# 0xPolygonZero/plonky2

Measured on AMD Instinct MI355X. Metric: LDE+Poseidon-commit GFE/s, higher is better.
Workload: dtype u64 (Goldilocks)

## Files before the change

### plonky2_amd/csrc/gl_mul3.hpp

```cpp
#pragma once
#include "asm_block.h"
#include "gl.hpp"

namespace gl {

#define P2_SA "v[70:71]", "v70", "v71", "v[72:73]", "v72", "v73", "v[74:75]", "v74", "v75", "s[40:41]", "s[42:43]"
#define P2_SB "v[76:77]", "v76", "v77", "v[78:79]", "v78", "v79", "v[80:81]", "v80", "v81", "s[44:45]", "s[46:47]"
#define P2_SC "v[82:83]", "v82", "v83", "v[84:85]", "v84", "v85", "v[86:87]", "v86", "v87", "s[48:49]", "s[50:51]"

#define P2_ST1(P, P0, P1, M, M0, M1, Q, Q0, Q1, C1, C2, a0, a1, b0, b1, r0, r1) "v_mad_u64_u32 " P ", " C1 ", %[" a0 "], %[" b0 "], 0\n\t"
#define P2_ST2(P, P0, P1, M, M0, M1, Q, Q0, Q1, C1, C2, a0, a1, b0, b1, r0, r1) "v_mad_u64_u32 " M ", " C1 ", %[" a1 "], %[" b0 "], 0\n\t"
#define P2_ST3(P, P0, P1, M, M0, M1, Q, Q0, Q1, C1, C2, a0, a1, b0, b1, r0, r1) "v_mad_u64_u32 " M ", " C2 ", %[" a0 "], %[" b1 "], " M "\n\t"
#define P2_ST4(P, P0, P1, M, M0, M1, Q, Q0, Q1, C1, C2, a0, a1, b0, b1, r0, r1) "v_mad_u64_u32 " Q ", " C1 ", %[" a1 "], %[" b1 "], 0\n\t"
#define P2_ST5(P, P0, P1, M, M0, M1, Q, Q0, Q1, C1, C2, a0, a1, b0, b1, r0, r1) "v_add_co_u32 " P1 ", " C1 ", " P1 ", " M0 "\n\t"
#define P2_ST6(P, P0, P1, M, M0, M1, Q, Q0, Q1, C1, C2, a0, a1, b0, b1, r0, r1) "v_addc_co_u32 " Q0 ", " C1 ", " Q0 ", " M1 ", " C1 "\n\t"
#define P2_ST7(P, P0, P1, M, M0, M1, Q, Q0, Q1, C1, C2, a0, a1, b0, b1, r0, r1) "v_addc_co_u32 " Q1 ", " C1 ", " Q1 ", 0, " C1 "\n\t"
#define P2_ST8(P, P0, P1, M, M0, M1, Q, Q0, Q1, C1, C2, a0, a1, b0, b1, r0, r1) "v_subb_co_u32 " P0 ", " C1 ", " P0 ", " Q1 ", " C2 "\n\t"
#define P2_ST9(P, P0, P1, M, M0, M1, Q, Q0, Q1, C1, C2, a0, a1, b0, b1, r0, r1) "v_subb_co_u32 " P1 ", " C1 ", " P1 ", 0, " C1 "\n\t"
#define P2_ST10(P, P0, P1, M, M0, M1, Q, Q0, Q1, C1, C2, a0, a1, b0, b1, r0, r1) "v_mad_u64_u32 " P ", " C2 ", " Q0 ", -1, " P "\n\t"
#define P2_ST11(P, P0, P1, M, M0, M1, Q, Q0, Q1, C1, C2, a0, a1, b0, b1, r0, r1) "v_cndmask_b32 " M0 ", 0, 1, " C2 "\n\t"
#define P2_ST12(P, P0, P1, M, M0, M1, Q, Q0, Q1, C1, C2, a0, a1, b0, b1, r0, r1) "v_subb_co_u32 " M0 ", " C1 ", " M0 ", 0, " C1 "\n\t"
#define P2_ST13(P, P0, P1, M, M0, M1, Q, Q0, Q1, C1, C2, a0, a1, b0, b1, r0, r1) "v_add_u32 " P1 ", " P1 ", " M0 "\n\t"
#define P2_ST14(P, P0, P1, M, M0, M1, Q, Q0, Q1, C1, C2, a0, a1, b0, b1, r0, r1) "v_mad_i64_i32 %[" r0 "], " C1 ", " M0 ", -1, " P "\n\t"

// ... 151 lines not shown
           (P2_CF_CLOBBERS3));
    r[0] = ra;
    r[1] = rb;
    r[2] = rc;
}

#define P2_CA1(ST) P2_APPLY(ST, P2_CA, "xa0", "xa1", "ya0", "ya1", "ra0")
__device__ __forceinline__ u64 mul1cf(u64 a, u64 b) {
    if (!P2_ASM_INTERPRETED()) return mul(a, b);
    u64 ra;
    P2_ASM(P2_CA1(P2_CF0) P2_CA1(P2_CF1) P2_CA1(P2_CF2) P2_CA1(P2_CF3) P2_CA1(P2_CF4) P2_CA1(P2_CF5) P2_CA1(P2_CF6) P2_CA1(P2_CF7)
               P2_CA1(P2_CF8) P2_CA1(P2_CF9) P2_NOP P2_CA1(P2_CF10) P2_CA1(P2_CF11) P2_NOP P2_CA1(P2_CF12) P2_CA1(P2_CF13)
                   P2_CA1(P2_CF14) P2_CA1(P2_CF15),
           (P2_O([ra0], "=&v", ra)),
           (P2_I([xa0], "v", (u32)a), P2_I([xa1], "v", (u32)(a >> 32)), P2_I([ya0], "v", (u32)b), P2_I([ya1], "v", (u32)(b >> 32))),
           ("v70", "v71", "v72", "v73", "v74", "v75", "v76", "v77", "s40", "s41", "s42", "s43"));
    return ra;
}

#define P2_CG0(P, P0, P1, M, M0, M1, N, N0, N1, T, T0, T1, C1, C2, a0, a1, b0, b1, r0) "v_mov_b32 " T1 ", 0\n\t"
#define P2_CG1(P, P0, P1, M, M0, M1, N, N0, N1, T, T0, T1, C1, C2, a0, a1, b0, b1, r0) "v_mad_u64_u32 " P ", " C1 ", %[" a0 "], %[" b0 "], 0\n\t"
#define P2_CG2(P, P0, P1, M, M0, M1, N, N0, N1, T, T0, T1, C1, C2, a0, a1, b0, b1, r0) "v_mov_b32 " T0 ", " P1 "\n\t"
#define P2_CG3(P, P0, P1, M, M0, M1, N, N0, N1, T, T0, T1, C1, C2, a0, a1, b0, b1, r0) "v_mad_u64_u32 " M ", " C1 ", %[" a1 "], %[" b0 "], " T "\n\t"
#define P2_CG4(P, P0, P1, M, M0, M1, N, N0, N1, T, T0, T1, C1, C2, a0, a1, b0, b1, r0) "v_mad_u64_u32 " N ", " C2 ", %[" a0 "], %[" b1 "], " M "\n\t"
#define P2_CG5(P, P0, P1, M, M0, M1, N, N0, N1, T, T0, T1, C1, C2, a0, a1, b0, b1, r0) "v_mov_b32 " T0 ", " N1 "\n\t"
#define P2_CG6(P, P0, P1, M, M0, M1, N, N0, N1, T, T0, T1, C1, C2, a0, a1, b0, b1, r0) "v_mad_u64_u32 " T ", " C1 ", %[" a1 "], %[" b1 "], " T "\n\t"
#define P2_CG7(P, P0, P1, M, M0, M1, N, N0, N1, T, T0, T1, C1, C2, a0, a1, b0, b1, r0) "v_subb_co_u32 " M0 ", " C1 ", " P0 ", " T1 ", " C2 "\n\t"
#define P2_CG8 P2_CF10
#define P2_CG9 P2_CF11
#define P2_CG10 P2_CF12
#define P2_CG11 P2_CF13
#define P2_CG12 P2_CF14
#define P2_CG13 P2_CF15

__device__ __forceinline__ void mul3cg(const u64 a[3], const u64 b[3], u64 r[3]) {
    if (!P2_ASM_INTERPRETED()) {
        for (int k = 0; k < 3; ++k) r[k] = mul(a[k], b[k]);
        return;
    }
    u64 ra, rb, rc;
    P2_ASM(P2_CROW(P2_CG0) P2_CROW(P2_CG1) P2_CROW(P2_CG2) P2_CROW(P2_CG3) P2_CROW(P2_CG4) P2_CROW(P2_CG5) P2_CROW(P2_CG6) P2_CROW(P2_CG7)
               P2_CROW(P2_CG8) P2_CROW(P2_CG9) P2_CROW(P2_CG10) P2_CROW(P2_CG11) P2_CROW(P2_CG12) P2_CROW(P2_CG13),
           (P2_O([ra0], "=&v", ra), P2_O([rb0], "=&v", rb), P2_O([rc0], "=&v", rc)),
           (P2_I([xa0], "v", (u32)a[0]), P2_I([xa1], "v", (u32)(a[0] >> 32)), P2_I([ya0], "v", (u32)b[0]),
            P2_I([ya1], "v", (u32)(b[0] >> 32)), P2_I([xb0], "v", (u32)a[1]), P2_I([xb1], "v", (u32)(a[1] >> 32)),
            P2_I([yb0], "v", (u32)b[1]), P2_I([yb1], "v", (u32)(b[1] >> 32)), P2_I([xc0], "v", (u32)a[2]),
            P2_I([xc1], "v", (u32)(a[2] >> 32)), P2_I([yc0], "v", (u32)b[2]), P2_I([yc1], "v", (u32)(b[2] >> 32))),
           (P2_CF_CLOBBERS3));
    r[0] = ra;
    r[1] = rb;
    r[2] = rc;
}

#define P2_HT "v[76:77]", "v76", "v77"
#define P2_HA "v[70:71]", "v70", "v71", "v[72:73]", "v72", "v73", "v[74:75]", "v74", "v75", P2_HT, "s[40:41]", "s[42:43]"
#define P2_HB "v[78:79]", "v78", "v79", "v[80:81]", "v80", "v81", "v[82:83]", "v82", "v83", P2_HT, "s[44:45]", "s[46:47]"
#define P2_HC "v[86:87]", "v86", "v87", "v[88:89]", "v88", "v89", "v[90:91]", "v90", "v91", P2_HT, "s[48:49]", "s[50:51]"
#define P2_CH23(...) P2_CG2(__VA_ARGS__) P2_CG3(__VA_ARGS__)
#define P2_CH6(P, P0, P1, M, M0, M1, N, N0, N1, T, T0, T1, C1, C2, a0, a1, b0, b1, r0) "v_mad_u64_u32 " M ", " C1 ", %[" a1 "], %[" b1 "], " T "\n\t"
#define P2_CH56(...) P2_CG5(__VA_ARGS__) P2_CH6(__VA_ARGS__)
#define P2_CH7(P, P0, P1, M, M0, M1, N, N0, N1, T, T0, T1, C1, C2, a0, a1, b0, b1, r0) "v_subb_co_u32 " P0 ", " C1 ", " P0 ", " M1 ", " C2 "\n\t"
#define P2_CH8(P, P0, P1, M, M0, M1, N, N0, N1, T, T0, T1, C1, C2, a0, a1, b0, b1, r0) "v_subb_co_u32 " P1 ", " C1 ", " N0 ", 0, " C1 "\n\t"
#define P2_CH9(P, P0, P1, M, M0, M1, N, N0, N1, T, T0, T1, C1, C2, a0, a1, b0, b1, r0) "v_mad_u64_u32 " P ", " C2 ", " M0 ", -1, " P "\n\t"
#define P2_CH12(P, P0, P1, M, M0, M1, N, N0, N1, T, T0, T1, C1, C2, a0, a1, b0, b1, r0) "v_add_u32 " P1 ", " P1 ", " N0 "\n\t"
#define P2_CH13(P, P0, P1, M, M0, M1, N, N0, N1, T, T0, T1, C1, C2, a0, a1, b0, b1, r0) "v_mad_i64_i32 %[" r0 "], " C1 ", " N0 ", -1, " P "\n\t"
#define P2_HROW(ST)                                          \
    P2_APPLY(ST, P2_HA, "xa0", "xa1", "ya0", "ya1", "ra0")   \
    P2_APPLY(ST, P2_HB, "xb0", "xb1", "yb0", "yb1", "rb0")   \
    P2_APPLY(ST, P2_HC, "xc0", "xc1", "yc0", "yc1", "rc0")
__device__ __forceinline__ void mul3ch(const u64 a[3], const u64 b[3], u64 r[3]) {
    if (!P2_ASM_INTERPRETED()) {
        for (int k = 0; k < 3; ++k) r[k] = mul(a[k], b[k]);
        return;
    }
    u64 ra, rb, rc;
    P2_ASM("v_mov_b32 v77, 0\n\t" P2_HROW(P2_CG1) P2_HROW(P2_CH23) P2_HROW(P2_CG4) P2_HROW(P2_CH56) P2_HROW(P2_CH7) P2_HROW(P2_CH8)
               P2_HROW(P2_CH9) P2_HROW(P2_CG10) P2_HROW(P2_CG11) P2_HROW(P2_CH12) P2_HROW(P2_CH13),
           (P2_O([ra0], "=&v", ra), P2_O([rb0], "=&v", rb), P2_O([rc0], "=&v", rc)),
           (P2_I([xa0], "v", (u32)a[0]), P2_I([xa1], "v", (u32)(a[0] >> 32)), P2_I([ya0], "v", (u32)b[0]),
            P2_I([ya1], "v", (u32)(b[0] >> 32)), P2_I([xb0], "v", (u32)a[1]), P2_I([xb1], "v", (u32)(a[1] >> 32)),
            P2_I([yb0], "v", (u32)b[1]), P2_I([yb1], "v", (u32)(b[1] >> 32)), P2_I([xc0], "v", (u32)a[2]),
            P2_I([xc1], "v", (u32)(a[2] >> 32)), P2_I([yc0], "v", (u32)b[2]), P2_I([yc1], "v", (u32)(b[2] >> 32))),
           ("v70", "v71", "v72", "v73", "v74", "v75", "v76", "v77", "v78", "v79", "v80", "v81", "v82", "v83", "v86", "v87", "v88", "v89",
            "v90", "v91", "s40", "s41", "s42", "s43", "s44", "s45", "s46", "s47", "s48", "s49", "s50", "s51"));
    r[0] = ra;
    r[1] = rb;
    r[2] = rc;
}

__device__ __forceinline__ u64 mul1cg(u64 a, u64 b) {
    if (!P2_ASM_INTERPRETED()) return mul(a, b);
    u64 ra;
    P2_ASM(P2_CA1(P2_CG0) P2_CA1(P2_CG1) P2_CA1(P2_CG2) P2_CA1(P2_CG3) P2_CA1(P2_CG4) P2_CA1(P2_CG5) P2_CA1(P2_CG6) P2_CA1(P2_CG7) P2_NOP
               P2_CA1(P2_CG8) P2_CA1(P2_CG9) P2_NOP P2_CA1(P2_CG10) P2_CA1(P2_CG11) P2_CA1(P2_CG12) P2_CA1(P2_CG13),
           (P2_O([ra0], "=&v", ra)),
           (P2_I([xa0], "v", (u32)a), P2_I([xa1], "v", (u32)(a >> 32)), P2_I([ya0], "v", (u32)b), P2_I([ya1], "v", (u32)(b >> 32))),
           ("v70", "v71", "v72", "v73", "v74", "v75", "v76", "v77", "s40", "s41", "s42", "s43"));
    return ra;
}

#define P2_FD1(P, P0, P1, M, M0, M1, Q, Q0, Q1, C1, C2, a0, a1, b0, b1, r0, r1) "v_mad_u64_u32 " P ", " C1 ", %[" b1 "], -1, %[" a0 "]\n\t"
#define P2_FD2(P, P0, P1, M, M0, M1, Q, Q0, Q1, C1, C2, a0, a1, b0, b1, r0, r1) "v_add_co_u32 " P1 ", " C1 ", " P1 ", %[" b0 "]\n\t"
#define P2_FD3(P, P0, P1, M, M0, M1, Q, Q0, Q1, C1, C2, a0, a1, b0, b1, r0, r1) "v_cndmask_b32 " M0 ", 0, -1, " C1 "\n\t"
#define P2_FD4(P, P0, P1, M, M0, M1, Q, Q0, Q1, C1, C2, a0, a1, b0, b1, r0, r1) "v_mad_u64_u32 %[" r0 "], " C1 ", " M0 ", 1, " P "\n\t"

__host__ __device__ __forceinline__ u64 fold_row_c(u64 al, u64 ah) {
    u32 k1;
    u32 w1 = addc32((u32)(al >> 32), (u32)ah, 0u, &k1);
    u32 w2 = (u32)(ah >> 32) + k1;
    u64 lo64 = ((u64)w1 << 32) | (u32)al;
    u64 t = (u64)w2 * 0xFFFFFFFFu + lo64;
    return fold_carry(t, t < lo64);
}

__device__ __forceinline__ void fold3(const u64 al[3], const u64 ah[3], u64 y[3]) {
    if (!P2_ASM_INTERPRETED()) {
        for (int k = 0; k < 3; ++k) y[k] = fold_row_c(al[k], ah[k]);
        return;
    }
    u64 ra, rb, rc;
    P2_ASM(P2_ROW(P2_FD1) P2_ROW(P2_FD2) P2_ROW(P2_FD3) P2_ROW(P2_FD4),
           (P2_O([ra0], "=&v", ra), P2_O([rb0], "=&v", rb), P2_O([rc0], "=&v", rc)),
           (P2_I([xa0], "v", al[0]), P2_I([ya0], "v", (u32)ah[0]), P2_I([ya1], "v", (u32)(ah[0] >> 32)),
            P2_I([xb0], "v", al[1]), P2_I([yb0], "v", (u32)ah[1]), P2_I([yb1], "v", (u32)(ah[1] >> 32)),
            P2_I([xc0], "v", al[2]), P2_I([yc0], "v", (u32)ah[2]), P2_I([yc1], "v", (u32)(ah[2] >> 32))),
           ("v70", "v71", "v72", "v76", "v77", "v78", "v82", "v83", "v84", "s40", "s41", "s44", "s45", "s48", "s49"));
    y[0] = ra;
    y[1] = rb;
    y[2] = rc;
}
__device__ __forceinline__ void fold2(const u64 al[2], const u64 ah[2], u64 y[2]) {
    if (!P2_ASM_INTERPRETED()) {
        for (int k = 0; k < 2; ++k) y[k] = fold_row_c(al[k], ah[k]);
        return;
    }
    u64 ra, rb;
    P2_ASM(P2_ROW2(P2_FD1) P2_ROW2(P2_FD2) P2_NOP0 P2_ROW2(P2_FD3) P2_ROW2(P2_FD4),
           (P2_O([ra0], "=&v", ra), P2_O([rb0], "=&v", rb)),
           (P2_I([xa0], "v", al[0]), P2_I([ya0], "v", (u32)ah[0]), P2_I([ya1], "v", (u32)(ah[0] >> 32)),
            P2_I([xb0], "v", al[1]), P2_I([yb0], "v", (u32)ah[1]), P2_I([yb1], "v", (u32)(ah[1] >> 32))),
           ("v70", "v71", "v72", "v76", "v77", "v78", "s40", "s41", "s44", "s45"));
    y[0] = ra;
    y[1] = rb;
}
__device__ __forceinline__ u64 fold1(u64 al, u64 ah) {
    if (!P2_ASM_INTERPRETED()) return fold_row_c(al, ah);
    u64 ra;
    P2_ASM(P2_A1(P2_FD1, P2_SA) P2_A1(P2_FD2, P2_SA) P2_NOP P2_A1(P2_FD3, P2_SA) P2_A1(P2_FD4, P2_SA),
           (P2_O([ra0], "=&v", ra)), (P2_I([xa0], "v", al), P2_I([ya0], "v", (u32)ah), P2_I([ya1], "v", (u32)(ah >> 32))),
           ("v70", "v71", "v72", "s40", "s41"));
    return ra;
}

}
```

### plonky2_amd/csrc/merkle.hpp

```cpp
#pragma once
#include "poseidon.hpp"
#include "poseidon4.hpp"
#include "poseidon16.hpp"
#include "ntt.hpp"

namespace merkle {
using gl::u32;
using gl::u64;

struct ColMajorReader {
    const u64 *m;
    size_t stride;
    __device__ __forceinline__ u64 operator()(size_t L, unsigned e) const { return m[(size_t)e * stride + L]; }
};
struct RowMajorReader {
    const u64 *m;
    size_t W;
    __device__ __forceinline__ u64 operator()(size_t L, unsigned e) const { return m[L * W + e]; }
};
struct FriPlanarReader {
    const u64 *p0, *p1;
    unsigned arity_bits;
    __device__ __forceinline__ u64 operator()(size_t L, unsigned e) const {
        const u64 *p = (e & 1) ? p1 : p0;
// ... 108 lines not shown
            }
            poseidon4::permute_quad(w, q);
        }
    }
    if (live) {
        u64 *dst = node_slot(digests, cap, h, 0, L);
        if (q == 0) {
            dst[0] = gl::canon(w[0]);
            dst[1] = gl::canon(w[1]);
            dst[2] = gl::canon(w[2]);
        } else if (q == 1) {
            dst[3] = gl::canon(w[0]);
        }
    }
}

__global__ void __launch_bounds__(256) merkle_level_quad_kernel(u64 *digests, u64 *cap, unsigned h, unsigned level,
                                                               size_t n_nodes) {
    const size_t j = ((size_t)blockIdx.x * blockDim.x + threadIdx.x) >> 2;
    const unsigned q = threadIdx.x & 3;
    const bool live = j < n_nodes;
    const u64 *ch = node_slot(digests, cap, h, level - 1, 2 * (live ? j : 0));
    u64 w[3];
#pragma unroll
    for (unsigned u = 0; u < 3; ++u) w[u] = (live && 3 * q + u < 8) ? ch[3 * q + u] : 0;
    poseidon4::permute_quad(w, q);
    if (live) {
        u64 *dst = node_slot(digests, cap, h, level, j);
        if (q == 0) {
            dst[0] = gl::canon(w[0]);
            dst[1] = gl::canon(w[1]);
            dst[2] = gl::canon(w[2]);
        } else if (q == 1) {
            dst[3] = gl::canon(w[0]);
        }
    }
}

template <class Reader>
__global__ void __launch_bounds__(256) hash_leaves_row_kernel(Reader rd, unsigned W, size_t leaf_offset, size_t leaf_count,
                                                             unsigned h, u64 *digests, u64 *cap) {
    const size_t t = ((size_t)blockIdx.x * blockDim.x + threadIdx.x) >> 4;
    const unsigned r = threadIdx.x & 15;
    const bool live = t < leaf_count;
    const size_t L = leaf_offset + (live ? t : 0);
    u64 w = 0;
    if (W <= 4) {
        if (live && r < W) w = rd(L, r);
    } else {
        const poseidon16::RowConsts k = poseidon16::row_consts(r);
        for (unsigned off = 0; off < W; off += 8) {
            const unsigned cnt = W - off < 8 ? W - off : 8;
            if (live && r < cnt) w = rd(L, off + r);
            poseidon16::permute_row(w, r, k);
        }
    }
    if (live && r < 4) node_slot(digests, cap, h, 0, L)[r] = gl::canon(w);
}

__global__ void __launch_bounds__(256) merkle_level_row_kernel(u64 *digests, u64 *cap, unsigned h, unsigned level, size_t n_nodes) {
    const size_t j = ((size_t)blockIdx.x * blockDim.x + threadIdx.x) >> 4;
    const unsigned r = threadIdx.x & 15;
    const bool live = j < n_nodes;
    const u64 *ch = node_slot(digests, cap, h, level - 1, 2 * (live ? j : 0));
    u64 w = (live && r < 8) ? ch[r] : 0;
    const poseidon16::RowConsts k = poseidon16::row_consts(r);
    poseidon16::permute_row(w, r, k);
    if (live && r < 4) node_slot(digests, cap, h, level, j)[r] = gl::canon(w);
}

__global__ void __launch_bounds__(256) permute_batch_row_kernel(u64 *states, size_t count) {
    const size_t t = ((size_t)blockIdx.x * blockDim.x + threadIdx.x) >> 4;
    const unsigned r = threadIdx.x & 15;
    const bool live = t < count && r < 12;
    u64 w = live ? states[12 * t + r] : 0;
    const poseidon16::RowConsts k = poseidon16::row_consts(r);
    poseidon16::permute_row(w, r, k);
    if (live) states[12 * t + r] = gl::canon(w);
}

__global__ void permute_batch_kernel(u64 *states, size_t count) {
    size_t t = (size_t)blockIdx.x * blockDim.x + threadIdx.x;
    if (t >= count) return;
    u64 s[12];
#pragma unroll
    for (int i = 0; i < 12; ++i) s[i] = states[12 * t + i];
    poseidon::permute(s);
#pragma unroll
    for (int i = 0; i < 12; ++i) states[12 * t + i] = gl::canon(s[i]);
}

__global__ void field_selftest_kernel(const u64 *a, const u64 *b, size_t count, u64 *out) {
    size_t t = (size_t)blockIdx.x * blockDim.x + threadIdx.x;
    if (t >= count) return;
    const u64 x = a[t], y = b[t];
    out[t] = gl::canon(gl::mul(x, y));
    out[count + t] = gl::canon(gl::mul1(x, y));
    u64 aa[3] = {x, y, x}, bb[3] = {y, x, x}, rr[3];
    gl::mul3(aa, bb, rr);
    u64 ok = (gl::canon(rr[1]) == gl::canon(rr[0])) && (gl::canon(rr[2]) == gl::canon(gl::mul(x, x))) ? 0 : 1;
    if (gl::canon(gl::mul1_lowregs(x, y)) != gl::canon(gl::mul(x, y))) ok |= 2;
#define P2_CHK_POW2(S)                                                                                              \
    if (gl::canon(ntt::mul_pow2_asm<S>(x)) != gl::canon(gl::mul(x, (S) < 64 ? 1ull << ((S) & 63) : 0xFFFFFFFFull << (((S) - 64) & 31)))) \
        ok |= 4;
    P2_CHK_POW2(12) P2_CHK_POW2(24) P2_CHK_POW2(36) P2_CHK_POW2(48) P2_CHK_POW2(60) P2_CHK_POW2(72) P2_CHK_POW2(84)
    P2_CHK_POW2(1) P2_CHK_POW2(31) P2_CHK_POW2(33) P2_CHK_POW2(63) P2_CHK_POW2(65) P2_CHK_POW2(95)
#undef P2_CHK_POW2
    {
        const u64 al = x >> 1, ah = y >> 1;
        const u64 want = gl::canon(gl::add(al, gl::mul(ah, 1ull << 32)));
        if (gl::canon(gl::fold1(al, ah)) != want) ok |= 8;
        const u64 al3[3] = {al, ah, al ^ 0x2AAAAAAAAAAAAAAAull}, ah3[3] = {ah, al, ah};
        u64 y3[3];
        gl::fold3(al3, ah3, y3);
        for (int k = 0; k < 3; ++k)
            if (gl::canon(y3[k]) != gl::canon(gl::add(al3[k], gl::mul(ah3[k], 1ull << 32)))) ok |= 16;
    }
    {
        const u64 a2[2] = {x, y ^ 0x9E3779B97F4A7C15ull}, b2[2] = {y, x};
        u64 r2[2];
        gl::mul2(a2, b2, r2);
        if (gl::canon(r2[0]) != gl::canon(gl::mul(x, y)) || gl::canon(r2[1]) != gl::canon(gl::mul(a2[1], x))) ok |= 32;
        const u64 l2[2] = {x >> 1, y >> 1}, h2[2] = {y >> 1, x >> 1};
        u64 f2[2];
        gl::fold2(l2, h2, f2);
        for (int k = 0; k < 2; ++k)
            if (gl::canon(f2[k]) != gl::canon(gl::add(l2[k], gl::mul(h2[k], 1ull << 32)))) ok |= 64;
    }
    if (gl::canon(gl::mul_add(x, y, x ^ y)) != gl::canon(gl::add(gl::mul(x, y), x ^ y)) || gl::canon(gl::mul_add(y, x, ~0ull)) != gl::canon(gl::add(gl::mul(x, y), ~0ull)) ||
        gl::canon(gl::mul_add(x, x, y)) != gl::canon(gl::add(gl::mul(x, x), y)))
        ok |= 128;
    {
        const u64 a3[3] = {x, y, x}, b3[3] = {y, x, x}, c3[3] = {x ^ y, ~0ull, y};
        u64 r3[3];
        gl::mad3(a3, b3, c3, r3);
        for (int k = 0; k < 3; ++k)
            if (gl::canon(r3[k]) != gl::canon(gl::add(gl::mul(a3[k], b3[k]), c3[k]))) ok |= 256;
    }
    {
        const u64 a3[3] = {x, y, x ^ 0x9E3779B97F4A7C15ull}, b3[3] = {y, y, x};
        u64 r3[3];
        gl::mul3cf(a3, b3, r3);
        for (int k = 0; k < 3; ++k)
            if (gl::canon(r3[k]) != gl::canon(gl::mul(a3[k], b3[k]))) ok |= 512;
        if (gl::canon(gl::mul1cf(x, y)) != gl::canon(gl::mul(x, y)) || gl::canon(gl::mul1cf(y, y)) != gl::canon(gl::mul(y, y))) ok |= 512;
        gl::mul3cg(a3, b3, r3);
        for (int k = 0; k < 3; ++k)
            if (gl::canon(r3[k]) != gl::canon(gl::mul(a3[k], b3[k]))) ok |= 512;
        gl::mul3ch(a3, b3, r3);
        for (int k = 0; k < 3; ++k)
            if (gl::canon(r3[k]) != gl::canon(gl::mul(a3[k], b3[k]))) ok |= 512;
        if (gl::canon(gl::mul1cg(x, y)) != gl::canon(gl::mul(x, y)) || gl::canon(gl::mul1cg(y, y)) != gl::canon(gl::mul(y, y))) ok |= 512;
    }
    out[2 * count + t] = gl::canon(rr[0]);
    out[5 * count + t] = ok;
    out[3 * count + t] = gl::canon(gl::add(x, y));
    out[4 * count + t] = gl::canon(gl::sub(x, y));
}

}
```

### plonky2_amd/csrc/poseidon.hpp

```cpp
#pragma once
#include "gl.hpp"
#include "gl_mul3.hpp"
#ifndef P2HOT_EMU
#define P2_CONST_QUAL __constant__
#endif
#define P2_LITERAL_QUAL static constexpr
#include "poseidon_constants.h"

namespace poseidon {
using gl::u32;
using gl::u64;

#define RC P2_POSEIDON_ALL_ROUND_CONSTANTS
#define RC_SPLIT P2_POSEIDON_PUSHED_ROUND_CONSTANTS_SPLIT

__device__ __forceinline__ u64 sbox7(u64 x) {
    u64 x2 = gl::sqr(x);
    u64 x4 = gl::sqr(x2);
    u64 x3 = gl::mul(x, x2);
    return gl::mul(x3, x4);
}

#ifndef P2HOT_SBOX_CF
#define P2HOT_SBOX_CF 2
// ... 67 lines not shown
        ah[0] += (u64)h0 * C;
        al[1] += (u64)l1 * C;
        ah[1] += (u64)h1 * C;
        al[2] += (u64)l2 * C;
        ah[2] += (u64)h2 * C;
        return;
    }
    u64 d;
    P2_ASM_NC("v_mad_u64_u32 %0, %6, %7, %13, %0\n\t"
              "v_mad_u64_u32 %1, %6, %8, %13, %1\n\t"
              "v_mad_u64_u32 %2, %6, %9, %13, %2\n\t"
              "v_mad_u64_u32 %3, %6, %10, %13, %3\n\t"
              "v_mad_u64_u32 %4, %6, %11, %13, %4\n\t"
              "v_mad_u64_u32 %5, %6, %12, %13, %5",
              (P2_O(, "+v", al[0]), P2_O(, "+v", ah[0]), P2_O(, "+v", al[1]), P2_O(, "+v", ah[1]), P2_O(, "+v", al[2]),
               P2_O(, "+v", ah[2]), P2_O(, "=&s", d)),
              (P2_I(, "v", l0), P2_I(, "v", h0), P2_I(, "v", l1), P2_I(, "v", h1), P2_I(, "v", l2), P2_I(, "v", h2),
               P2_I(, "n", C)));
}
template <bool HAS_K>
__device__ __forceinline__ void mds_first(u64 (&al)[3], u64 (&ah)[3], u32 l0, u32 h0, u32 l1, u32 h1, u32 l2, u32 h2,
                                          const u64 *k) {
    if (!P2_ASM_INTERPRETED()) {
        const u64 z[6] = {0, 0, 0, 0, 0, 0};
        const u64 *kk = HAS_K ? k : z;
        al[0] = (u64)l0 * 17u + kk[0];
        ah[0] = (u64)h0 * 17u + kk[1];
        al[1] = (u64)l1 * 17u + kk[2];
        ah[1] = (u64)h1 * 17u + kk[3];
        al[2] = (u64)l2 * 17u + kk[4];
        ah[2] = (u64)h2 * 17u + kk[5];
        return;
    }
    u64 d;
    if (HAS_K) {
        P2_ASM_NC("v_mad_u64_u32 %0, %6, %7, 17, %13\n\t"
                  "v_mad_u64_u32 %1, %6, %8, 17, %14\n\t"
                  "v_mad_u64_u32 %2, %6, %9, 17, %15\n\t"
                  "v_mad_u64_u32 %3, %6, %10, 17, %16\n\t"
                  "v_mad_u64_u32 %4, %6, %11, 17, %17\n\t"
                  "v_mad_u64_u32 %5, %6, %12, 17, %18",
                  (P2_O(, "=&v", al[0]), P2_O(, "=&v", ah[0]), P2_O(, "=&v", al[1]), P2_O(, "=&v", ah[1]),
                   P2_O(, "=&v", al[2]), P2_O(, "=&v", ah[2]), P2_O(, "=&s", d)),
                  (P2_I(, "v", l0), P2_I(, "v", h0), P2_I(, "v", l1), P2_I(, "v", h1), P2_I(, "v", l2), P2_I(, "v", h2),
                   P2_I(, "s", k[0]), P2_I(, "s", k[1]), P2_I(, "s", k[2]), P2_I(, "s", k[3]), P2_I(, "s", k[4]),
                   P2_I(, "s", k[5])));
    } else {
        P2_ASM_NC("v_mad_u64_u32 %0, %6, %7, 17, 0\n\t"
                  "v_mad_u64_u32 %1, %6, %8, 17, 0\n\t"
                  "v_mad_u64_u32 %2, %6, %9, 17, 0\n\t"
                  "v_mad_u64_u32 %3, %6, %10, 17, 0\n\t"
                  "v_mad_u64_u32 %4, %6, %11, 17, 0\n\t"
                  "v_mad_u64_u32 %5, %6, %12, 17, 0",
                  (P2_O(, "=&v", al[0]), P2_O(, "=&v", ah[0]), P2_O(, "=&v", al[1]), P2_O(, "=&v", ah[1]),
                   P2_O(, "=&v", al[2]), P2_O(, "=&v", ah[2]), P2_O(, "=&s", d)),
                  (P2_I(, "v", l0), P2_I(, "v", h0), P2_I(, "v", l1), P2_I(, "v", h1), P2_I(, "v", l2), P2_I(, "v", h2)));
    }
}

template <int R>
__device__ __forceinline__ u64 mds_row(const u32 (&xl)[12], const u32 (&xh)[12]) {
    static_assert(R > 0 && R < 12, "row 0 carries the diagonal term");
    constexpr u32 C[12] = {17, 15, 41, 16, 2, 28, 13, 13, 39, 18, 34, 20};
    u64 al = (u64)xl[R] * opaque_const(C[0]), ah = (u64)xh[R] * opaque_const(C[0]);
#pragma unroll
    for (int i = 1; i < 12; ++i) {
        al += (u64)xl[(R + i) % 12] * opaque_const(C[i]);
        ah += (u64)xh[(R + i) % 12] * opaque_const(C[i]);
    }
    return gl::fold1(al, ah);
}

__device__ __forceinline__ void mds_layer(u64 s[12], const u64 *rc2, unsigned groups = 0xFu, int single = -1) {
    u32 xl[12], xh[12];
#pragma unroll
    for (int i = 0; i < 12; ++i) {
        xl[i] = (u32)s[i];
        xh[i] = (u32)(s[i] >> 32);
    }
#pragma unroll
    for (int g = 0; g < 12; g += 3) {
        if (!(groups >> (g / 3) & 1u)) continue;
        u64 al[3], ah[3], y[3];
#define P2_X(i) xl[(g + (i)) % 12], xh[(g + (i)) % 12], xl[(g + (i) + 1) % 12], xh[(g + (i) + 1) % 12], xl[(g + (i) + 2) % 12], xh[(g + (i) + 2) % 12]
        if (rc2)
            mds_first<true>(al, ah, P2_X(0), rc2 + 2 * g);
        else
            mds_first<false>(al, ah, P2_X(0), nullptr);
        mds_term<15>(al, ah, P2_X(1));
        mds_term<41>(al, ah, P2_X(2));
        mds_term<16>(al, ah, P2_X(3));
        mds_term<2>(al, ah, P2_X(4));
        mds_term<28>(al, ah, P2_X(5));
        mds_term<13>(al, ah, P2_X(6));
        mds_term<13>(al, ah, P2_X(7));
        mds_term<39>(al, ah, P2_X(8));
        mds_term<18>(al, ah, P2_X(9));
        mds_term<34>(al, ah, P2_X(10));
        mds_term<20>(al, ah, P2_X(11));
#undef P2_X
        if (g == 0) {
            al[0] += (u64)xl[0] * opaque_const(8);
            ah[0] += (u64)xh[0] * opaque_const(8);
        }
        gl::fold3(al, ah, y);
        s[g] = y[0];
        s[g + 1] = y[1];
        s[g + 2] = y[2];
    }
    if (single == 3)
        s[3] = mds_row<3>(xl, xh);
    else if (single == 8)
        s[8] = mds_row<8>(xl, xh);
}

struct Mat12 {
    u32 v[144];
};
constexpr Mat12 mds_matrix() {
    Mat12 m{};
    for (int r = 0; r < 12; ++r)
        for (int c = 0; c < 12; ++c) m.v[12 * r + c] = P2_POSEIDON_M1_ROW0[(c - r + 12) % 12] - ((c - r + 12) % 12 == 0 ? 8u : 0u) + (r == 0 && c == 0 ? 8u : 0u);
    return m;
}
constexpr Mat12 mat_mul(const Mat12 &a, const Mat12 &b) {
    Mat12 m{};
    for (int r = 0; r < 12; ++r)
        for (int c = 0; c < 12; ++c) {
            u64 acc = 0;
            for (int k = 0; k < 12; ++k) acc += (u64)a.v[12 * r + k] * b.v[12 * k + c];
            m.v[12 * r + c] = (u32)acc;
        }
    return m;
}
constexpr bool mat_checks() {
    const Mat12 m1 = mds_matrix(), m2 = mat_mul(m1, m1), m3 = mat_mul(m1, m2);
    for (int j = 0; j < 12; ++j) {
        if (m1.v[j] != P2_POSEIDON_M1_ROW0[j] || m2.v[j] != P2_POSEIDON_M2_ROW0[j]) return false;
        if (m1.v[12 * j] != P2_POSEIDON_MCOL0[j] || m2.v[12 * j] != P2_POSEIDON_MCOL0[12 + j]) return false;
    }
    for (int i = 0; i < 144; ++i)
        if (m3.v[i] != P2_POSEIDON_M3[i]) return false;
    return true;
}
static_assert(mat_checks(), "M, M^2, M^3: the compile-time products disagree with the generated tables");
constexpr Mat12 mat_drop_col0(const Mat12 &a) {
    Mat12 m = a;
    for (int r = 0; r < 12; ++r) m.v[12 * r] = 0;
    return m;
}
P2_LITERAL_QUAL Mat12 MDS1 = mds_matrix();
P2_LITERAL_QUAL Mat12 MDM = mat_mul(mat_drop_col0(mds_matrix()), mds_matrix());
P2_LITERAL_QUAL Mat12 MDMDM = mat_mul(mat_drop_col0(mds_matrix()), mat_mul(mat_drop_col0(mds_matrix()), mds_matrix()));

__device__ __forceinline__ void mds_partial_round(u64 s[12], u64 c, u64 cn) {
    u32 xl[12], xh[12];
#pragma unroll
    for (int i = 0; i < 12; ++i) {
        xl[i] = (u32)s[i];
        xh[i] = (u32)(s[i] >> 32);
    }
    u64 al = (u32)c, ah = c >> 32;
#pragma unroll
    for (int j = 0; j < 12; ++j) {
        al += (u64)xl[j] * P2_POSEIDON_M1_ROW0[j];
        ah += (u64)xh[j] * P2_POSEIDON_M1_ROW0[j];
    }
    const u64 s1 = sbox7_asm(gl::fold1(al, ah));
    const u32 sl = (u32)s1, sh = (u32)(s1 >> 32);
#pragma unroll
    for (int g = 0; g < 12; g += 3) {
        u64 bl[3], bh[3], y[3];
#pragma unroll
        for (int t = 0; t < 3; ++t) {
            const int i = g + t;
            bl[t] = (u64)sl * MDS1.v[12 * i] + (i == 0 ? (u64)(u32)cn : 0);
            bh[t] = (u64)sh * MDS1.v[12 * i] + (i == 0 ? cn >> 32 : 0);
#pragma unroll
            for (int j = 0; j < 12; ++j) {
                bl[t] += (u64)xl[j] * MDM.v[12 * i + j];
                bh[t] += (u64)xh[j] * MDM.v[12 * i + j];
            }
        }
        gl::fold3(bl, bh, y);
        s[g] = y[0];
        s[g + 1] = y[1];
        s[g + 2] = y[2];
    }
}

template <bool TAIL = false>
__device__ __forceinline__ void partial_rounds3(u64 s[12], u64 c1, u64 c2, u64 cn, const u64 *cv = nullptr) {
    u32 xl[12], xh[12];
    const u64 z0 = sbox7_asm(s[0]);
    xl[0] = (u32)z0;
    xh[0] = (u32)(z0 >> 32);
#pragma unroll
    for (int i = 1; i < 12; ++i) {
        xl[i] = (u32)s[i];
        xh[i] = (u32)(s[i] >> 32);
    }
    u64 al = (u32)c1, ah = c1 >> 32;
#pragma unroll
    for (int j = 0; j < 12; ++j) {
        al += (u64)xl[j] * P2_POSEIDON_M1_ROW0[j];
        ah += (u64)xh[j] * P2_POSEIDON_M1_ROW0[j];
    }
    const u64 s1 = sbox7_asm(gl::fold1(al, ah));
    const u32 s1l = (u32)s1, s1h = (u32)(s1 >> 32);
    al = (u64)s1l * MDS1.v[0] + (u32)c2;
    ah = (u64)s1h * MDS1.v[0] + (c2 >> 32);
#pragma unroll
    for (int j = 0; j < 12; ++j) {
        al += (u64)xl[j] * MDM.v[j];
        ah += (u64)xh[j] * MDM.v[j];
    }
    const u64 s2 = sbox7_asm(gl::fold1(al, ah));
    const u32 s2l = (u32)s2, s2h = (u32)(s2 >> 32);
#pragma unroll
    for (int g = 0; g < 12; g += 3) {
        u64 bl[3], bh[3], y[3];
#pragma unroll
        for (int t = 0; t < 3; ++t) {
            const int i = g + t;
            const u64 ci = TAIL ? cv[i] : (i == 0 ? cn : 0);
            bl[t] = (u64)s1l * MDM.v[12 * i] + (u64)s2l * MDS1.v[12 * i] + (u32)ci;
            bh[t] = (u64)s1h * MDM.v[12 * i] + (u64)s2h * MDS1.v[12 * i] + (ci >> 32);
#pragma unroll
            for (int j = 0; j < 12; ++j) {
                bl[t] += (u64)xl[j] * MDMDM.v[12 * i + j];
                bh[t] += (u64)xh[j] * MDMDM.v[12 * i + j];
            }
        }
        gl::fold3(bl, bh, y);
        s[g] = y[0];
        s[g + 1] = y[1];
        s[g + 2] = y[2];
    }
}

#ifndef P2HOT_TAIL_BATCH
#define P2HOT_TAIL_BATCH 1
#endif
__device__ inline void permute(u64 s[12], unsigned out_groups = 0xFu, int out_single = -1) {
    const u32 z0 = opaque_zero();
#pragma unroll
    for (int i = 0; i < 12; ++i) s[i] = ark(s[i], RC[i + z0]);
    int round = 0;
#pragma unroll 1
    for (int k = 0; k < 3; ++k, ++round) {
        sbox_layer(s);
        mds_layer(s, RC_SPLIT + 24 * (round + 1));
    }
    sbox_layer(s);
    mds_partial_round(s, P2_POSEIDON_PUSHED_ROUND_CONSTANTS[12 * 4], P2_POSEIDON_PUSHED_ROUND_CONSTANTS[12 * 5]);
    round = 5;
#pragma unroll 1
    for (int k = 0; k < (P2HOT_TAIL_BATCH ? 6 : 7); ++k, round += 3)
        partial_rounds3(s, P2_POSEIDON_PUSHED_ROUND_CONSTANTS[12 * (round + 1)], P2_POSEIDON_PUSHED_ROUND_CONSTANTS[12 * (round + 2)],
                        P2_POSEIDON_PUSHED_ROUND_CONSTANTS[12 * (round + 3)]);
    const u32 z26 = opaque_zero();
    if (P2HOT_TAIL_BATCH) {
        partial_rounds3<true>(s, P2_POSEIDON_PUSHED_ROUND_CONSTANTS[12 * 24], P2_POSEIDON_PUSHED_ROUND_CONSTANTS[12 * 25], 0,
                              P2_POSEIDON_PUSHED_ROUND_CONSTANTS + 12 * 26 + z26);
        round = 26;
    } else {
#pragma unroll
        for (int i = 1; i < 12; ++i) s[i] = ark(s[i], P2_POSEIDON_PUSHED_ROUND_CONSTANTS[12 * round + i + z26]);
    }
#pragma unroll 1
    for (int k = 0; k < 3; ++k, ++round) {
        sbox_layer(s);
        mds_layer(s, RC_SPLIT + 24 * (round + 1));
    }
    sbox_layer(s);
    mds_layer(s, nullptr, out_groups, out_single);
}

__device__ __forceinline__ void two_to_one(const u64 l[4], const u64 r[4], u64 out[4]) {
    u64 s[12];
#pragma unroll
    for (int i = 0; i < 4; ++i) {
        s[i] = l[i];
        s[4 + i] = r[i];
        s[8 + i] = 0;
    }
    permute(s, 0x1u, 3);
#pragma unroll
    for (int i = 0; i < 4; ++i) out[i] = gl::canon(s[i]);
}

#undef RC
#undef RC_SPLIT
}
```

Measured before the change: 20.53.

## Batch Poseidon partial rounds four at a time with wide fold

Replaces the single-round mds_partial_round plus partial_rounds3 batches with a partial_rounds4 routine. It chains three scalar sboxes through precomputed (MD)^k M matrices, so one full 12-wide matrix pass covers four partial rounds. A new fold3w/fold1w reduction handles the larger accumulator rows, and a static_assert checks at compile time that the 64-bit chains cannot overflow. The aim is fewer full 12x12 dense MDS passes per permutation, at the cost of more scalar dot products per batch and possibly higher register pressure.

```diff
diff --git a/plonky2_amd/csrc/gl_mul3.hpp b/plonky2_amd/csrc/gl_mul3.hpp
--- a/plonky2_amd/csrc/gl_mul3.hpp
+++ b/plonky2_amd/csrc/gl_mul3.hpp
@@ -327,4 +327,44 @@
     return ra;
 }
 
-}
+#define P2_FW1(P, P0, P1, M, M0, M1, Q, Q0, Q1, C1, C2, a0, a1, b0, b1, r0, r1) "v_mad_u64_u32 " P ", " C1 ", %[" b1 "], -1, %[" a0 "]\n\t"
+#define P2_FW2(P, P0, P1, M, M0, M1, Q, Q0, Q1, C1, C2, a0, a1, b0, b1, r0, r1) "v_cndmask_b32 " M0 ", 0, -1, " C1 "\n\t"
+#define P2_FW3(P, P0, P1, M, M0, M1, Q, Q0, Q1, C1, C2, a0, a1, b0, b1, r0, r1) "v_mad_u64_u32 " P ", " C1 ", " M0 ", 1, " P "\n\t"
+#define P2_FW4 P2_FD2
+#define P2_FW5 P2_FD3
+#define P2_FW6 P2_FD4
+
+__host__ __device__ __forceinline__ u64 fold_row_wide_c(u64 al, u64 ah) {
+    u64 t = (ah >> 32) * 0xFFFFFFFFull + al;
+    t += t < al ? 0xFFFFFFFFull : 0;
+    const u64 u = t + (ah << 32);
+    return u + (u < t ? 0xFFFFFFFFull : 0);
+}
+
+__device__ __forceinline__ void fold3w(const u64 al[3], const u64 ah[3], u64 y[3]) {
+    if (!P2_ASM_INTERPRETED()) {
+        for (int k = 0; k < 3; ++k) y[k] = fold_row_wide_c(al[k], ah[k]);
+        return;
+    }
+    u64 ra, rb, rc;
+    P2_ASM(P2_ROW(P2_FW1) P2_ROW(P2_FW2) P2_ROW(P2_FW3) P2_ROW(P2_FW4) P2_ROW(P2_FW5) P2_ROW(P2_FW6),
+           (P2_O([ra0], "=&v", ra), P2_O([rb0], "=&v", rb), P2_O([rc0], "=&v", rc)),
+           (P2_I([xa0], "v", al[0]), P2_I([ya0], "v", (u32)ah[0]), P2_I([ya1], "v", (u32)(ah[0] >> 32)),
+            P2_I([xb0], "v", al[1]), P2_I([yb0], "v", (u32)ah[1]), P2_I([yb1], "v", (u32)(ah[1] >> 32)),
+            P2_I([xc0], "v", al[2]), P2_I([yc0], "v", (u32)ah[2]), P2_I([yc1], "v", (u32)(ah[2] >> 32))),
+           ("v70", "v71", "v72", "v76", "v77", "v78", "v82", "v83", "v84", "s40", "s41", "s44", "s45", "s48", "s49"));
+    y[0] = ra;
+    y[1] = rb;
+    y[2] = rc;
+}
+__device__ __forceinline__ u64 fold1w(u64 al, u64 ah) {
+    if (!P2_ASM_INTERPRETED()) return fold_row_wide_c(al, ah);
+    u64 ra;
+    P2_ASM(P2_A1(P2_FW1, P2_SA) P2_NOP P2_A1(P2_FW2, P2_SA) P2_A1(P2_FW3, P2_SA) P2_A1(P2_FW4, P2_SA) P2_NOP P2_A1(P2_FW5, P2_SA)
+               P2_A1(P2_FW6, P2_SA),
+           (P2_O([ra0], "=&v", ra)), (P2_I([xa0], "v", al), P2_I([ya0], "v", (u32)ah), P2_I([ya1], "v", (u32)(ah >> 32))),
+           ("v70", "v71", "v72", "s40", "s41"));
+    return ra;
+}
+
+}
diff --git a/plonky2_amd/csrc/merkle.hpp b/plonky2_amd/csrc/merkle.hpp
--- a/plonky2_amd/csrc/merkle.hpp
+++ b/plonky2_amd/csrc/merkle.hpp
@@ -284,6 +284,14 @@
             if (gl::canon(r3[k]) != gl::canon(gl::mul(a3[k], b3[k]))) ok |= 512;
         if (gl::canon(gl::mul1cg(x, y)) != gl::canon(gl::mul(x, y)) || gl::canon(gl::mul1cg(y, y)) != gl::canon(gl::mul(y, y))) ok |= 512;
     }
+    {
+        const u64 al3[3] = {x, y, x ^ y}, ah3[3] = {y, x, ~x};
+        u64 y3[3];
+        gl::fold3w(al3, ah3, y3);
+        for (int k = 0; k < 3; ++k)
+            if (gl::canon(y3[k]) != gl::canon(gl::add(al3[k], gl::mul(ah3[k], 1ull << 32)))) ok |= 1024;
+        if (gl::canon(gl::fold1w(x, y)) != gl::canon(gl::add(x, gl::mul(y, 1ull << 32)))) ok |= 1024;
+    }
     out[2 * count + t] = gl::canon(rr[0]);
     out[5 * count + t] = ok;
     out[3 * count + t] = gl::canon(gl::add(x, y));
diff --git a/plonky2_amd/csrc/poseidon.hpp b/plonky2_amd/csrc/poseidon.hpp
--- a/plonky2_amd/csrc/poseidon.hpp
+++ b/plonky2_amd/csrc/poseidon.hpp
@@ -243,37 +243,79 @@
 P2_LITERAL_QUAL Mat12 MDS1 = mds_matrix();
 P2_LITERAL_QUAL Mat12 MDM = mat_mul(mat_drop_col0(mds_matrix()), mds_matrix());
 P2_LITERAL_QUAL Mat12 MDMDM = mat_mul(mat_drop_col0(mds_matrix()), mat_mul(mat_drop_col0(mds_matrix()), mds_matrix()));
-
-__device__ __forceinline__ void mds_partial_round(u64 s[12], u64 c, u64 cn) {
+P2_LITERAL_QUAL Mat12 MDMDMDM = mat_mul(mat_drop_col0(mds_matrix()), MDMDM);
+
+constexpr bool pass4_rows_fit() {
+    const Mat12 m1 = mds_matrix(), md = mat_drop_col0(m1);
+    const Mat12 p1 = mat_mul(md, m1), p2 = mat_mul(md, p1), p3 = mat_mul(md, p2);
+    for (int i = 0; i < 144; ++i)
+        if (p1.v[i] != MDM.v[i] || p2.v[i] != MDMDM.v[i] || p3.v[i] != MDMDMDM.v[i]) return false;
+    for (int r = 0; r < 12; ++r) {
+        u64 sum = (u64)p2.v[12 * r] + p1.v[12 * r] + m1.v[12 * r];
+        for (int c = 0; c < 12; ++c) {
+            u64 e = 0;
+            for (int k = 0; k < 12; ++k) e += (u64)md.v[12 * r + k] * p2.v[12 * k + c];
+            if (e != p3.v[12 * r + c]) return false;
+            sum += e;
+        }
+        if (sum > (1ull << 32)) return false;
+    }
+    return true;
+}
+static_assert(pass4_rows_fit(), "(MD)^3 M: a four-application row would overflow its 64-bit chains");
+
+template <bool FIRST = false>
+__device__ __forceinline__ void partial_rounds4(u64 s[12], u64 c1, u64 c2, u64 c3, u64 cn) {
     u32 xl[12], xh[12];
-#pragma unroll
-    for (int i = 0; i < 12; ++i) {
+    const u64 z0 = FIRST ? s[0] : sbox7_asm(s[0]);
+    xl[0] = (u32)z0;
+    xh[0] = (u32)(z0 >> 32);
+#pragma unroll
+    for (int i = 1; i < 12; ++i) {
         xl[i] = (u32)s[i];
         xh[i] = (u32)(s[i] >> 32);
     }
-    u64 al = (u32)c, ah = c >> 32;
+    u64 al = (u32)c1, ah = c1 >> 32;
 #pragma unroll
     for (int j = 0; j < 12; ++j) {
         al += (u64)xl[j] * P2_POSEIDON_M1_ROW0[j];
         ah += (u64)xh[j] * P2_POSEIDON_M1_ROW0[j];
     }
     const u64 s1 = sbox7_asm(gl::fold1(al, ah));
-    const u32 sl = (u32)s1, sh = (u32)(s1 >> 32);
+    const u32 s1l = (u32)s1, s1h = (u32)(s1 >> 32);
+    al = (u64)s1l * MDS1.v[0] + (u32)c2;
+    ah = (u64)s1h * MDS1.v[0] + (c2 >> 32);
+#pragma unroll
+    for (int j = 0; j < 12; ++j) {
+        al += (u64)xl[j] * MDM.v[j];
+        ah += (u64)xh[j] * MDM.v[j];
+    }
+    const u64 s2 = sbox7_asm(gl::fold1(al, ah));
+    const u32 s2l = (u32)s2, s2h = (u32)(s2 >> 32);
+    al = (u64)s1l * MDM.v[0] + (u64)s2l * MDS1.v[0] + (u32)c3;
+    ah = (u64)s1h * MDM.v[0] + (u64)s2h * MDS1.v[0] + (c3 >> 32);
+#pragma unroll
+    for (int j = 0; j < 12; ++j) {
+        al += (u64)xl[j] * MDMDM.v[j];
+        ah += (u64)xh[j] * MDMDM.v[j];
+    }
+    const u64 s3 = sbox7_asm(gl::fold1(al, ah));
+    const u32 s3l = (u32)s3, s3h = (u32)(s3 >> 32);
 #pragma unroll
     for (int g = 0; g < 12; g += 3) {
         u64 bl[3], bh[3], y[3];
 #pragma unroll
         for (int t = 0; t < 3; ++t) {
             const int i = g + t;
-            bl[t] = (u64)sl * MDS1.v[12 * i] + (i == 0 ? (u64)(u32)cn : 0);
-            bh[t] = (u64)sh * MDS1.v[12 * i] + (i == 0 ? cn >> 32 : 0);
+            bl[t] = (u64)s1l * MDMDM.v[12 * i] + (u64)s2l * MDM.v[12 * i] + (u64)s3l * MDS1.v[12 * i] + (i == 0 ? (u64)(u32)cn : 0);
+            bh[t] = (u64)s1h * MDMDM.v[12 * i] + (u64)s2h * MDM.v[12 * i] + (u64)s3h * MDS1.v[12 * i] + (i == 0 ? cn >> 32 : 0);
 #pragma unroll
             for (int j = 0; j < 12; ++j) {
-                bl[t] += (u64)xl[j] * MDM.v[12 * i + j];
-                bh[t] += (u64)xh[j] * MDM.v[12 * i + j];
+                bl[t] += (u64)xl[j] * MDMDMDM.v[12 * i + j];
+                bh[t] += (u64)xh[j] * MDMDMDM.v[12 * i + j];
             }
         }
-        gl::fold3(bl, bh, y);
+        gl::fold3w(bl, bh, y);
         s[g] = y[0];
         s[g + 1] = y[1];
         s[g + 2] = y[2];
@@ -344,21 +386,24 @@
         mds_layer(s, RC_SPLIT + 24 * (round + 1));
     }
     sbox_layer(s);
-    mds_partial_round(s, P2_POSEIDON_PUSHED_ROUND_CONSTANTS[12 * 4], P2_POSEIDON_PUSHED_ROUND_CONSTANTS[12 * 5]);
-    round = 5;
+    partial_rounds4<true>(s, P2_POSEIDON_PUSHED_ROUND_CONSTANTS[12 * 4], P2_POSEIDON_PUSHED_ROUND_CONSTANTS[12 * 5],
+                          P2_POSEIDON_PUSHED_ROUND_CONSTANTS[12 * 6], P2_POSEIDON_PUSHED_ROUND_CONSTANTS[12 * 7]);
+    round = 7;
 #pragma unroll 1
-    for (int k = 0; k < (P2HOT_TAIL_BATCH ? 6 : 7); ++k, round += 3)
-        partial_rounds3(s, P2_POSEIDON_PUSHED_ROUND_CONSTANTS[12 * (round + 1)], P2_POSEIDON_PUSHED_ROUND_CONSTANTS[12 * (round + 2)],
-                        P2_POSEIDON_PUSHED_ROUND_CONSTANTS[12 * (round + 3)]);
+    for (int k = 0; k < 4; ++k, round += 4)
+        partial_rounds4(s, P2_POSEIDON_PUSHED_ROUND_CONSTANTS[12 * (round + 1)], P2_POSEIDON_PUSHED_ROUND_CONSTANTS[12 * (round + 2)],
+                        P2_POSEIDON_PUSHED_ROUND_CONSTANTS[12 * (round + 3)], P2_POSEIDON_PUSHED_ROUND_CONSTANTS[12 * (round + 4)]);
     const u32 z26 = opaque_zero();
     if (P2HOT_TAIL_BATCH) {
         partial_rounds3<true>(s, P2_POSEIDON_PUSHED_ROUND_CONSTANTS[12 * 24], P2_POSEIDON_PUSHED_ROUND_CONSTANTS[12 * 25], 0,
                               P2_POSEIDON_PUSHED_ROUND_CONSTANTS + 12 * 26 + z26);
-        round = 26;
     } else {
-#pragma unroll
-        for (int i = 1; i < 12; ++i) s[i] = ark(s[i], P2_POSEIDON_PUSHED_ROUND_CONSTANTS[12 * round + i + z26]);
-    }
+        partial_rounds3(s, P2_POSEIDON_PUSHED_ROUND_CONSTANTS[12 * 24], P2_POSEIDON_PUSHED_ROUND_CONSTANTS[12 * 25],
+                        P2_POSEIDON_PUSHED_ROUND_CONSTANTS[12 * 26]);
+#pragma unroll
+        for (int i = 1; i < 12; ++i) s[i] = ark(s[i], P2_POSEIDON_PUSHED_ROUND_CONSTANTS[12 * 26 + i + z26]);
+    }
+    round = 26;
 #pragma unroll 1
     for (int k = 0; k < 3; ++k, ++round) {
         sbox_layer(s);
```

Result: faster. 21.17 (median of 6 runs) (+3.1%).
